# uber-research/UPSNet

Hardware: AMD Instinct MI355X
Metric: images/sec (whole node), UPSNet-50 1024x2048 (higher is better)
Workload: dtype f32

## Files before the change

upsnet_amd/csrc/conv_wino36.hip:

```cpp
#include <cstdlib>
#include <type_traits>
#include "conv_params.h"
#include "upsnet_hip.h"

#define W36_TM 32
#define W36_TN 64
#define W36_PTS 36
#define W36_VBUF (W36_PTS * 4 * W36_TM * 16)
#define W36_BSTEP (2 * W36_TN * 16)
#define W36_STEPS (2 * W36_PTS)
#define W36_XCH (16 * W36_PTS * 64 * 4)
#define W36_RING 3

typedef unsigned w36_uintx4 __attribute__((ext_vector_type(4)));

#define W36_BT(D0, D1, D2, D3, D4, D5)                                                                               \
    {                                                                                                                \
        const float a0_ = D0, a1_ = D1, a2_ = D2, a3_ = D3, a4_ = D4, a5_ = D5;                                       \
        const float e1_ = __builtin_fmaf(-2.25f, a2_, a4_), o1_ = __builtin_fmaf(-2.25f, a1_, a3_);                   \
        const float e3_ = __builtin_fmaf(-0.5625f, a2_, a4_), o3_ = __builtin_fmaf(-0.5625f, a1_, a3_);               \
        D0 = __builtin_fmaf(1.265625f, a0_, __builtin_fmaf(-2.8125f, a2_, a4_));                                     \
        D1 = __builtin_fmaf(0.75f, o1_, e1_);                                                                        \
        D2 = __builtin_fmaf(-0.75f, o1_, e1_);                                                                       \
        D3 = __builtin_fmaf(1.5f, o3_, e3_);                                                                         \
        D4 = __builtin_fmaf(-1.5f, o3_, e3_);                                                                        \
        D5 = __builtin_fmaf(1.265625f, a1_, __builtin_fmaf(-2.8125f, a3_, a5_));                                     \
    }
#define W36_AT(M0, M1, M2, M3, M4, M5, Y0, Y1, Y2, Y3)                                                               \
    {                                                                                                                \
        const float s1_ = (M1) + (M2), d1_ = (M1) - (M2), s2_ = (M3) + (M4), d2_ = (M3) - (M4);                      \
        Y0 = ((M0) + s1_) + s2_;                                                                                     \
        Y1 = __builtin_fmaf(1.5f, d2_, 0.75f * d1_);                                                                 \
        Y2 = __builtin_fmaf(2.25f, s2_, 0.5625f * s1_);                                                              \
        Y3 = __builtin_fmaf(3.375f, d2_, __builtin_fmaf(0.421875f, d1_, (M5)));                                      \
    }

template <bool SK>
__global__ void __launch_bounds__(512, 1) conv_wino36_f32_kernel(const ConvParams p)
{
    extern __shared__ __attribute__((aligned(16))) unsigned char smem_raw[];
    const int tid = threadIdx.x, lane = tid & 63;
    const int wave = __builtin_amdgcn_readfirstlane(tid >> 6);
    const int cb = wave >> 2, pg = wave & 3;
    const int lhalf = lane >> 5, l32 = lane & 31;
    int m_t, n_t, kz = 0;
    {
        const int nt = p.n_tiles;
        const int per = (p.m_tiles + 7) >> 3;
        int bid = (int)blockIdx.x;
        if constexpr (SK) { const int base_grid = 8 * per * nt; kz = bid / base_grid; bid -= kz * base_grid; }
        const int q = bid >> 3;
        n_t = q % nt;
        const int local = q / nt;
        m_t = (bid & 7) * per + local;
        if (local >= per || m_t >= p.m_tiles) return;
    }
    int si = 0;
#pragma unroll
    for (int q = 1; q < CV_MAXSEG; ++q) if (q < p.nseg && m_t >= p.seg[q].tile_start) si = q;
    const ConvSeg sg = p.seg[si];
    const long p0 = (long)(m_t - sg.tile_start) * W36_TM;
    const int nslabs_all = p.Cin >> 4;
    const int s_first = SK ? (kz * nslabs_all) / p.ksplit : 0;
    const int nslabs = SK ? ((kz + 1) * nslabs_all) / p.ksplit - s_first : nslabs_all;
    const long HoWo = (long)sg.Ho * sg.Wo;

    const int ltile = tid >> 4, lch = tid & 15;
    int hrow0, wcol0;
    int hlo, hhi;
    unsigned tbase, nrmask = 0, ncmask = 0;
    bool lane_fix;
    {
        const long pp = p0 + ltile;
        const bool tile_ok = pp < sg.M;
        const long ppc = tile_ok ? pp : sg.M - 1;
        const int n = (int)(ppc / HoWo);
        const int rem = (int)(ppc - (long)n * HoWo);
        const int ty = rem / sg.Wo, tx = rem - ty * sg.Wo;
        const int h0 = 4 * ty - 1;
        hlo = n * sg.H; hhi = tile_ok ? hlo + sg.H : hlo;
        hrow0 = hlo + h0;
        wcol0 = 4 * tx - 1;
#pragma unroll
        for (int r = 0; r < 6; ++r) nrmask |= (h0 + r >= 0 && h0 + r < sg.H) ? 0u : (1u << r);
#pragma unroll
        for (int c = 0; c < 6; ++c) ncmask |= (wcol0 + c >= 0 && wcol0 + c < sg.W) ? 0u : (1u << c);
        lane_fix = tile_ok && (nrmask | ncmask) != 0;
        tbase = (unsigned)(hrow0 * sg.W + wcol0) * (4u * (unsigned)p.Cin) + 4u * (unsigned)lch;
    }
    const bool fix = __builtin_amdgcn_ballot_w64(lane_fix) != 0ull;
    bool risky;
    {
        const long plast = min(p0 + (long)W36_TM, sg.M) - 1;
        const long nl = plast / HoWo;
        const long tyl = (plast - nl * HoWo) / sg.Wo;
        risky = (nl * sg.H + 4 * tyl + 4) * (long)sg.W + 4L * sg.Wo >= (long)sg.N * sg.H * sg.W;
    }
    const unsigned cin4 = 4u * (unsigned)p.Cin;
    const unsigned rowpitch = (unsigned)sg.W * cin4;
    const unsigned cin4_s = __builtin_amdgcn_readfirstlane(cin4);
    const unsigned rowpitch_s = __builtin_amdgcn_readfirstlane((unsigned)sg.W) * cin4_s;
    const unsigned cbase = (unsigned)wcol0 * cin4 + 4u * (unsigned)lch;
#define W36_ROWOFF(R) (((unsigned)min(max(hrow0 + (R), hlo), max(hhi - 1, hlo)) * rowpitch) | ((hrow0 + (R) >= hlo && hrow0 + (R) < hhi) ? 0u : 0x80000000u))
    const size_t xaddr = reinterpret_cast<size_t>(sg.x);
    const unsigned xlo = __builtin_amdgcn_readfirstlane((unsigned)xaddr), xhi = __builtin_amdgcn_readfirstlane((unsigned)(xaddr >> 32));
    const unsigned xbytes = __builtin_amdgcn_readfirstlane((unsigned)(sg.N * sg.H * sg.W) * 4u * (unsigned)p.Cin - (SK ? (unsigned)s_first * 64u : 0u));
    const char *xbase = reinterpret_cast<const char *>(((size_t)xhi << 32) | xlo) + (SK ? (size_t)s_first * 64 : 0);
#define W36_SWZ(Q) ((((Q) & 1) << 2) | (((Q) >> 1) << 1))
    const unsigned st_base = (unsigned)((((lch >> 2) * W36_TM + (ltile ^ W36_SWZ(lch >> 2))) * 16) + (lch & 3) * 4);
    constexpr unsigned XI_PITCH = 4 * W36_TM * 16;
    const unsigned fr_base0 = (unsigned)((lhalf * W36_TM + (l32 ^ W36_SWZ(lhalf))) * 16) + (unsigned)pg * 9u * XI_PITCH;
    const unsigned fr_base1 = (unsigned)(((2 + lhalf) * W36_TM + (l32 ^ W36_SWZ(2 + lhalf))) * 16) + (unsigned)pg * 9u * XI_PITCH;
    const size_t waddr = reinterpret_cast<size_t>(p.w) + ((size_t)n_t * (size_t)nslabs_all + (size_t)s_first) * (W36_STEPS * W36_BSTEP);
    const unsigned wlo = __builtin_amdgcn_readfirstlane((unsigned)waddr), whi = __builtin_amdgcn_readfirstlane((unsigned)(waddr >> 32));
    const __amdgpu_buffer_rsrc_t wrsrc = __builtin_amdgcn_make_buffer_rsrc(reinterpret_cast<void *>(((size_t)whi << 32) | wlo), 0,
                                                                            nslabs * (int)(W36_STEPS * W36_BSTEP), 0x00020000);
    const unsigned b_lane = (unsigned)(lhalf * (W36_TN * 16) + (32 * cb + l32) * 16);
    const int gmax = nslabs * W36_STEPS - 1;

    floatx16 acc[9];
#pragma unroll
    for (int i = 0; i < 9; ++i)
#pragma unroll
        for (int r = 0; r < 16; ++r) acc[i][r] = 0.f;

    float ld[36];
    float4 breg[W36_RING];

#define W36_LOADROW_FAST(R, RS) { unsigned so_ = (unsigned)((R) ? (R) - 1 : 0) * rowpitch_s; asm volatile("" : "+s"(so_));              \
        ld[6 * (R)] = __uint_as_float(__builtin_amdgcn_raw_buffer_load_b32(RS, (R) ? tbase + rowpitch_s : tbase, so_, 0));               \
        _Pragma("unroll") for (int c_ = 1; c_ < 6; ++c_) ld[6 * (R) + c_] = __uint_as_float(__builtin_amdgcn_raw_buffer_load_b32(       \
            RS, ((R) ? tbase + rowpitch_s : tbase) + cin4_s, so_ + (unsigned)(c_ - 1) * cin4_s, 0)); }
#define W36_LOADROW_SAFE(R, RS) { unsigned cb_ = cbase; asm volatile("" : "+v"(cb_)); const unsigned rb_ = W36_ROWOFF(R) + cb_; _Pragma("unroll") for (int c_ = 0; c_ < 6; ++c_) \
        ld[6 * (R) + c_] = __uint_as_float(__builtin_amdgcn_raw_buffer_load_b32(RS, (rb_ + (unsigned)c_ * cin4) | ((ncmask << (30 - c_)) & 0x40000000u), 0, 0)); }
#define W36_FIXROW(R) if (fix) { asm volatile("" ::: "memory"); const unsigned bad_ = ((nrmask >> (R)) & 1u) ? 0x3fu : ncmask;           \
        _Pragma("unroll") for (int c_ = 0; c_ < 6; ++c_) ld[6 * (R) + c_] = ((bad_ >> c_) & 1u) ? 0.f : ld[6 * (R) + c_]; }
#define W36_ROWPASS(R) W36_BT(ld[6 * (R) + 0], ld[6 * (R) + 1], ld[6 * (R) + 2], ld[6 * (R) + 3], ld[6 * (R) + 4], ld[6 * (R) + 5])
#define W36_COLSTASH(J, SB)                                                                                           \
    {                                                                                                                 \
        float c0_ = ld[0 + (J)], c1_ = ld[6 + (J)], c2_ = ld[12 + (J)], c3_ = ld[18 + (J)], c4_ = ld[24 + (J)], c5_ = ld[30 + (J)]; \
        W36_BT(c0_, c1_, c2_, c3_, c4_, c5_)                                                                          \
        *reinterpret_cast<float *>(smem_raw + (SB) + (0 * 6 + (J)) * XI_PITCH) = c0_;                                 \
        *reinterpret_cast<float *>(smem_raw + (SB) + (1 * 6 + (J)) * XI_PITCH) = c1_;                                 \
        *reinterpret_cast<float *>(smem_raw + (SB) + (2 * 6 + (J)) * XI_PITCH) = c2_;                                 \
        *reinterpret_cast<float *>(smem_raw + (SB) + (3 * 6 + (J)) * XI_PITCH) = c3_;                                 \
        *reinterpret_cast<float *>(smem_raw + (SB) + (4 * 6 + (J)) * XI_PITCH) = c4_;                                 \
        *reinterpret_cast<float *>(smem_raw + (SB) + (5 * 6 + (J)) * XI_PITCH) = c5_;                                 \
    }
#define W36_BLOAD(SLOT, G) { const w36_uintx4 v_ = __builtin_amdgcn_raw_buffer_load_b128(wrsrc, b_lane, (unsigned)min((G), gmax) * W36_BSTEP, 0); \
        breg[SLOT] = make_float4(__uint_as_float(v_.x), __uint_as_float(v_.y), __uint_as_float(v_.z), __uint_as_float(v_.w)); }

#pragma unroll
    for (int u = 0; u < W36_RING; ++u) W36_BLOAD(u, 18 * pg + u)
    {
        const __amdgpu_buffer_rsrc_t xr = __builtin_amdgcn_make_buffer_rsrc(const_cast<char *>(xbase), 0, xbytes, 0x00020000);
#pragma unroll
        for (int r = 0; r < 6; ++r) { W36_LOADROW_SAFE(r, xr) }
#pragma unroll
        for (int r = 0; r < 6; ++r) { W36_ROWPASS(r) }
#pragma unroll
        for (int j = 0; j < 6; ++j) { W36_COLSTASH(j, st_base) }
    }
    __syncthreads();
    float4 afr = *reinterpret_cast<const float4 *>(smem_raw + fr_base0);

    auto slab_loop = [&](auto fast_tag) __attribute__((always_inline)) {
    constexpr bool FAST = decltype(fast_tag)::value;
    for (int s = 0; s < nslabs; ++s) {
        const int sn = min(s + 1, nslabs - 1);
        const __amdgpu_buffer_rsrc_t xr = __builtin_amdgcn_make_buffer_rsrc(const_cast<char *>(xbase) + (size_t)sn * 64, 0, xbytes - (unsigned)sn * 64u, 0x00020000);
        const unsigned cur = (s & 1) ? W36_VBUF : 0u, nxt = W36_VBUF - cur;
        const unsigned sb = nxt + st_base;
        const int g0 = s * W36_STEPS + 18 * pg;
#pragma unroll
        for (int u = 0; u < 18; ++u) {
            if (u < 6) { if constexpr (FAST) { W36_LOADROW_FAST(u, xr) } else { W36_LOADROW_SAFE(u, xr) } }
            float4 afn;
            if (u < 17) afn = *reinterpret_cast<const float4 *>(smem_raw + cur + (((u + 1) & 1) ? fr_base1 : fr_base0) + (unsigned)((u + 1) >> 1) * XI_PITCH);
            else afn = *reinterpret_cast<const float4 *>(smem_raw + nxt + fr_base0);
            if (u == 6) { if constexpr (FAST) { W36_FIXROW(0) } W36_ROWPASS(0) }
            if (u == 7) { if constexpr (FAST) { W36_FIXROW(1) } W36_ROWPASS(1) }
            if (u == 8) { if constexpr (FAST) { W36_FIXROW(2) } W36_ROWPASS(2) }
            if (u == 9) { if constexpr (FAST) { W36_FIXROW(3) } W36_ROWPASS(3) }
            if (u == 10) { if constexpr (FAST) { W36_FIXROW(4) } W36_ROWPASS(4) }
            if (u == 11) { if constexpr (FAST) { W36_FIXROW(5) } W36_ROWPASS(5) W36_COLSTASH(0, sb) }
            if (u == 12) { W36_COLSTASH(1, sb) }
            if (u == 13) { W36_COLSTASH(2, sb) }
            if (u == 14) { W36_COLSTASH(3, sb) }
            if (u == 15) { W36_COLSTASH(4, sb) }
            if (u == 16) { W36_COLSTASH(5, sb) }
            const float4 bf = breg[u % W36_RING];
            acc[u >> 1] = __builtin_amdgcn_mfma_f32_32x32x2f32(afr.x, bf.x, acc[u >> 1], 0, 0, 0);
            acc[u >> 1] = __builtin_amdgcn_mfma_f32_32x32x2f32(afr.y, bf.y, acc[u >> 1], 0, 0, 0);
            acc[u >> 1] = __builtin_amdgcn_mfma_f32_32x32x2f32(afr.z, bf.z, acc[u >> 1], 0, 0, 0);
            acc[u >> 1] = __builtin_amdgcn_mfma_f32_32x32x2f32(afr.w, bf.w, acc[u >> 1], 0, 0, 0);
            W36_BLOAD(u % W36_RING, (u + W36_RING < 18 ? g0 : g0 + W36_STEPS - 18) + u + W36_RING)
            if (u == 16) __syncthreads();
            afr = afn;
            __builtin_amdgcn_sched_barrier(0);
        }
    }
    };
    if (risky) slab_loop(std::false_type{}); else slab_loop(std::true_type{});
#undef W36_LOADROW_FAST
#undef W36_LOADROW_SAFE
#undef W36_ROWOFF
#undef W36_FIXROW
#undef W36_ROWPASS
#undef W36_COLSTASH
#undef W36_BLOAD

    const unsigned crow = (unsigned)p.Cout * 4u;
    const size_t oaddr_ = reinterpret_cast<size_t>(SK ? p.partial + (size_t)kz * (size_t)p.m_total * (size_t)p.Cout : sg.out);
    const unsigned obytes_ = __builtin_amdgcn_readfirstlane((unsigned)((long)sg.N * sg.OH * sg.OW) * crow);
    const __amdgpu_buffer_rsrc_t orsrc = __builtin_amdgcn_make_buffer_rsrc(
        reinterpret_cast<void *>(((size_t)(unsigned)__builtin_amdgcn_readfirstlane((unsigned)(oaddr_ >> 32)) << 32) | (unsigned)__builtin_amdgcn_readfirstlane((unsigned)oaddr_)),
        0, (int)obytes_, 0x00020000);
    float *xch = reinterpret_cast<float *>(smem_raw);
#pragma unroll 1
    for (int bb = 0; bb < 2; ++bb) {
        __syncthreads();
        if (cb == bb) {
#pragma unroll
            for (int u = 0; u < 9; ++u)
#pragma unroll
                for (int r = 0; r < 16; ++r) xch[(r * W36_PTS + 9 * pg + u) * 64 + lane] = acc[u][r];
        }
        __syncthreads();
        const int co_ch = n_t * W36_TN + 32 * bb + l32;
        const bool co_ok = co_ch < p.Cout;
        const float bv = (p.bias != nullptr && co_ok) ? p.bias[co_ch] : 0.f;
#pragma unroll 1
        for (int rr = 0; rr < 2; ++rr) {
            const int r = 2 * wave + rr;
            const long pp = p0 + 8 * (r >> 2) + 4 * lhalf + (r & 3);
            float m[36];
#pragma unroll
            for (int x = 0; x < 36; ++x) m[x] = xch[(r * W36_PTS + x) * 64 + lane];
            if (!(co_ok && pp < sg.M)) continue;
            const int n = (int)(pp / HoWo);
            const int rem = (int)(pp - (long)n * HoWo);
            const int ty = rem / sg.Wo, tx = rem - ty * sg.Wo;
            float t[6][4];
#pragma unroll
            for (int i = 0; i < 6; ++i) W36_AT(m[6 * i + 0], m[6 * i + 1], m[6 * i + 2], m[6 * i + 3], m[6 * i + 4], m[6 * i + 5], t[i][0], t[i][1], t[i][2], t[i][3])
#pragma unroll
            for (int c = 0; c < 4; ++c) {
                float y[4];
                W36_AT(t[0][c], t[1][c], t[2][c], t[3][c], t[4][c], t[5][c], y[0], y[1], y[2], y[3])
                const int ox = 4 * tx + c;
#pragma unroll
                for (int a = 0; a < 4; ++a) {
                    const int oy = 4 * ty + a;
                    float v = y[a];
                    if constexpr (!SK) { v = v + bv; if (p.relu) v = fmaxf(v, 0.f); }
                    const unsigned off = (oy < sg.OH && ox < sg.OW) ? (unsigned)((n * sg.OH + oy) * sg.OW + ox) * crow + 4u * (unsigned)co_ch : 0x80000000u;
                    __builtin_amdgcn_raw_buffer_store_b32(__float_as_uint(v), orsrc, off, 0, 0);
                }
            }
        }
    }
}

static int w36_fill(ConvParams &p, const char *who, int nseg, const float *const x[], float *const out[], const int batch[], const int height[],
                    const int width[], int Cin, int Cout, const float *wpack, int ldw, const float *bias, int relu)
{
    UPS_REQUIRE(Cin > 0 && Cin % 32 == 0 && ldw % W36_TN == 0, "%s: Cin %% 32 == 0 and ldw %% 64 == 0 (got %d, %d)", who, Cin, ldw);
    int rc = conv_fill(p, who, nseg, x, nullptr, nullptr, nullptr, out, batch, height, width, Cin, Cout, wpack, ldw, bias, 3, 3, 1, 1, 1, relu);
    if (rc) return rc;
    UPS_REQUIRE((long)W36_PTS * Cin * ldw < (1L << 29), "%s: packed weight exceeds 2 GiB", who);
    int tiles = 0;
    for (int i = 0; i < nseg; ++i) {
        ConvSeg &s = p.seg[i];
        s.OH = s.Ho; s.OW = s.Wo;
        s.Ho = (s.OH + 3) / 4; s.Wo = (s.OW + 3) / 4;
        s.M = (long)s.N * s.Ho * s.Wo;
        UPS_REQUIRE((long)s.N * s.H * s.W * Cin < (1L << 28), "%s: feature map %d exceeds 1 GiB; split the batch", who, i);
        UPS_REQUIRE((long)s.N * s.OH * s.OW * Cout < (1L << 29), "%s: output %d exceeds 2 GiB; split the batch", who, i);
        s.tile_start = tiles;
        tiles += (int)((s.M + W36_TM - 1) / W36_TM);
    }
    p.m_tiles = tiles;
    p.n_tiles = ldw / W36_TN;
    return 0;
}

extern "C" int upsnet_conv2d_winograd36_nhwc_f32(void *stream, int nseg, const float *const x[], float *const out[], const int batch[],
                                                 const int height[], const int width[], int Cin, const float *wpack, int ldw, const float *bias,
                                                 int Cout, int relu)
{
    ConvParams p;
    int rc = w36_fill(p, "conv2d_winograd36_nhwc_f32", nseg, x, out, batch, height, width, Cin, Cout, wpack, ldw, bias, relu);
    if (rc) return rc;
    static std::atomic<unsigned long long> attr_dev{0};
    UPS_ONCE_PER_DEVICE(attr_dev, UPS_CHECK_HIP(hipFuncSetAttribute(reinterpret_cast<const void *>(&conv_wino36_f32_kernel<false>), hipFuncAttributeMaxDynamicSharedMemorySize, W36_XCH)));
    const int grid = 8 * ((p.m_tiles + 7) / 8) * p.n_tiles;
    hipLaunchKernelGGL(conv_wino36_f32_kernel<false>, dim3(grid), dim3(512), W36_XCH, (hipStream_t)stream, p);
    UPS_CHECK_LAUNCH("conv_wino36_f32_kernel");
    ups_set_form("wino36<%d,%d>", W36_TM, W36_TN);
    return 0;
}

extern "C" size_t upsnet_conv2d_winograd36_splitk_workspace_bytes(int batch, int height, int width, int Cout, int ksplit)
{
    return (size_t)ksplit * (size_t)batch * height * width * Cout * sizeof(float);
}

extern "C" int upsnet_conv2d_winograd36_nhwc_f32_splitk(void *stream, const float *x, float *out, int batch, int height, int width, int Cin,
                                                        const float *wpack, int ldw, const float *bias, int Cout, int relu, int ksplit,
                                                        void *workspace)
{
    const float *xs[1] = {x};
    float *os[1] = {out};
    const int nb[1] = {batch}, hh[1] = {height}, ww[1] = {width};
    ConvParams p;
    int rc = w36_fill(p, "conv2d_winograd36_nhwc_f32_splitk", 1, xs, os, nb, hh, ww, Cin, Cout, wpack, ldw, bias, relu);
    if (rc) return rc;
    UPS_REQUIRE(workspace && ksplit >= 2 && ksplit <= 8 && Cin / 16 >= ksplit, "conv2d_winograd36_nhwc_f32_splitk: ksplit 2..8, <= Cin / 16, and a workspace");
    p.ksplit = ksplit;
    p.partial = (float *)workspace;
    p.m_total = (long)batch * height * width;
    UPS_REQUIRE(p.m_total * Cout < (1L << 29), "conv2d_winograd36_nhwc_f32_splitk: output exceeds 2 GiB; split the batch");
    static std::atomic<unsigned long long> attr_dev{0};
    UPS_ONCE_PER_DEVICE(attr_dev, UPS_CHECK_HIP(hipFuncSetAttribute(reinterpret_cast<const void *>(&conv_wino36_f32_kernel<true>), hipFuncAttributeMaxDynamicSharedMemorySize, W36_XCH)));
    const int grid = 8 * ((p.m_tiles + 7) / 8) * p.n_tiles * ksplit;
    hipLaunchKernelGGL(conv_wino36_f32_kernel<true>, dim3(grid), dim3(512), W36_XCH, (hipStream_t)stream, p);
    UPS_CHECK_LAUNCH("conv_wino36_f32_kernel<splitk>");
    ups_set_form("wino36<%d,%d> splitk%d", W36_TM, W36_TN, ksplit);
    return conv_splitk_reduce((hipStream_t)stream, p.partial, ksplit, p.m_total, p.m_total, Cout, bias, nullptr, relu, out);
}

__global__ void conv_pack_weight_wino36_kernel(const float *__restrict__ w, int cout, int cin, int ldw, float *__restrict__ wp)
{
    const long total = (long)ldw * cin;
    const int nslabs = cin >> 4;
    const double G[6][3] = {{64.0 / 81, 0.0, 0.0}, {-128.0 / 243, -32.0 / 81, -8.0 / 27}, {-128.0 / 243, 32.0 / 81, -8.0 / 27},
                            {32.0 / 243, 16.0 / 81, 8.0 / 27}, {32.0 / 243, -16.0 / 81, 8.0 / 27}, {0.0, 0.0, 1.0}};
    for (long idx = (long)blockIdx.x * blockDim.x + threadIdx.x; idx < total; idx += (long)blockDim.x * gridDim.x) {
        const int co = idx % ldw, c = idx / ldw;
        double g[3][3], t[6][3];
#pragma unroll
        for (int a = 0; a < 3; ++a)
#pragma unroll
            for (int b = 0; b < 3; ++b) g[a][b] = co < cout ? (double)w[(((long)co * cin + c) * 3 + a) * 3 + b] : 0.0;
#pragma unroll
        for (int i = 0; i < 6; ++i)
#pragma unroll
            for (int b = 0; b < 3; ++b) t[i][b] = G[i][0] * g[0][b] + G[i][1] * g[1][b] + G[i][2] * g[2][b];
        const long blk = ((long)(co / W36_TN) * nslabs + (c >> 4)) * W36_PTS;
        const int q = (c & 15) >> 2, ci = c & 3, cl = co % W36_TN;
#pragma unroll
        for (int i = 0; i < 6; ++i)
#pragma unroll
            for (int j = 0; j < 6; ++j) {
                const double u = t[i][0] * G[j][0] + t[i][1] * G[j][1] + t[i][2] * G[j][2];
                wp[(((blk + i * 6 + j) * 4 + q) * W36_TN + cl) * 4 + ci] = (float)u;
            }
    }
}

extern "C" int upsnet_conv_pack_weight_winograd36(void *stream, const float *weight, int cout, int cin, int ldw, float *wpack)
{
    UPS_REQUIRE(weight && wpack && cout > 0 && cin > 0 && ldw >= cout, "conv_pack_weight_winograd36: bad args");
    UPS_REQUIRE(cin % 16 == 0 && ldw % W36_TN == 0, "conv_pack_weight_winograd36: Cin %% 16 must be 0 and ldw a multiple of 64");
    const long total = (long)ldw * cin;
    int blocks = (int)((total + 255) / 256);
    if (blocks > 65535) blocks = 65535;
    hipLaunchKernelGGL(conv_pack_weight_wino36_kernel, dim3(blocks), dim3(256), 0, (hipStream_t)stream, weight, cout, cin, ldw, wpack);
    UPS_CHECK_LAUNCH("conv_pack_weight_wino36_kernel");
    return 0;
}
```

Baseline: 172.4.

## Restructure Winograd epilogue exchange layout, vectorize LDS traffic, use fast prologue loads

Reworks the output-transform epilogue: accumulators are written to LDS as float4 in a new interleaved layout, then read as float2 pairs so each lane handles two adjacent tiles. Tile index math is done once and incremented, and store offsets are hoisted per row. The prologue now uses the fast input-load path when the tile is not risky, and the column stash splits its high rows into a separate base address. The aim is fewer LDS instructions, less integer division, and cheaper address math, in exchange for higher register pressure and more complex indexing.

```diff
diff --git a/upsnet_amd/csrc/conv_wino36.hip b/upsnet_amd/csrc/conv_wino36.hip
--- a/upsnet_amd/csrc/conv_wino36.hip
+++ b/upsnet_amd/csrc/conv_wino36.hip
@@ -13,6 +13,7 @@
 #define W36_RING 3
 
 typedef unsigned w36_uintx4 __attribute__((ext_vector_type(4)));
+typedef float w36_floatx2 __attribute__((ext_vector_type(2)));
 
 #define W36_BT(D0, D1, D2, D3, D4, D5)                                                                               \
     {                                                                                                                \
@@ -136,7 +137,7 @@
 #define W36_FIXROW(R) if (fix) { asm volatile("" ::: "memory"); const unsigned bad_ = ((nrmask >> (R)) & 1u) ? 0x3fu : ncmask;           \
         _Pragma("unroll") for (int c_ = 0; c_ < 6; ++c_) ld[6 * (R) + c_] = ((bad_ >> c_) & 1u) ? 0.f : ld[6 * (R) + c_]; }
 #define W36_ROWPASS(R) W36_BT(ld[6 * (R) + 0], ld[6 * (R) + 1], ld[6 * (R) + 2], ld[6 * (R) + 3], ld[6 * (R) + 4], ld[6 * (R) + 5])
-#define W36_COLSTASH(J, SB)                                                                                           \
+#define W36_COLSTASH(J, SB, SBH)                                                                                      \
     {                                                                                                                 \
         float c0_ = ld[0 + (J)], c1_ = ld[6 + (J)], c2_ = ld[12 + (J)], c3_ = ld[18 + (J)], c4_ = ld[24 + (J)], c5_ = ld[30 + (J)]; \
         W36_BT(c0_, c1_, c2_, c3_, c4_, c5_)                                                                          \
@@ -144,8 +145,8 @@
         *reinterpret_cast<float *>(smem_raw + (SB) + (1 * 6 + (J)) * XI_PITCH) = c1_;                                 \
         *reinterpret_cast<float *>(smem_raw + (SB) + (2 * 6 + (J)) * XI_PITCH) = c2_;                                 \
         *reinterpret_cast<float *>(smem_raw + (SB) + (3 * 6 + (J)) * XI_PITCH) = c3_;                                 \
-        *reinterpret_cast<float *>(smem_raw + (SB) + (4 * 6 + (J)) * XI_PITCH) = c4_;                                 \
-        *reinterpret_cast<float *>(smem_raw + (SB) + (5 * 6 + (J)) * XI_PITCH) = c5_;                                 \
+        *reinterpret_cast<float *>(smem_raw + (SBH) + (J) * XI_PITCH) = c4_;                                          \
+        *reinterpret_cast<float *>(smem_raw + (SBH) + (6 + (J)) * XI_PITCH) = c5_;                                    \
     }
 #define W36_BLOAD(SLOT, G) { const w36_uintx4 v_ = __builtin_amdgcn_raw_buffer_load_b128(wrsrc, b_lane, (unsigned)min((G), gmax) * W36_BSTEP, 0); \
         breg[SLOT] = make_float4(__uint_as_float(v_.x), __uint_as_float(v_.y), __uint_as_float(v_.z), __uint_as_float(v_.w)); }
@@ -154,12 +155,20 @@
     for (int u = 0; u < W36_RING; ++u) W36_BLOAD(u, 18 * pg + u)
     {
         const __amdgpu_buffer_rsrc_t xr = __builtin_amdgcn_make_buffer_rsrc(const_cast<char *>(xbase), 0, xbytes, 0x00020000);
-#pragma unroll
-        for (int r = 0; r < 6; ++r) { W36_LOADROW_SAFE(r, xr) }
+        if (risky) {
+#pragma unroll
+            for (int r = 0; r < 6; ++r) { W36_LOADROW_SAFE(r, xr) }
+        } else {
+#pragma unroll
+            for (int r = 0; r < 6; ++r) { W36_LOADROW_FAST(r, xr) }
+#pragma unroll
+            for (int r = 0; r < 6; ++r) { W36_FIXROW(r) }
+        }
 #pragma unroll
         for (int r = 0; r < 6; ++r) { W36_ROWPASS(r) }
-#pragma unroll
-        for (int j = 0; j < 6; ++j) { W36_COLSTASH(j, st_base) }
+        const unsigned st_hi = st_base + 24u * XI_PITCH;
+#pragma unroll
+        for (int j = 0; j < 6; ++j) { W36_COLSTASH(j, st_base, st_hi) }
     }
     __syncthreads();
     float4 afr = *reinterpret_cast<const float4 *>(smem_raw + fr_base0);
@@ -171,6 +180,8 @@
         const __amdgpu_buffer_rsrc_t xr = __builtin_amdgcn_make_buffer_rsrc(const_cast<char *>(xbase) + (size_t)sn * 64, 0, xbytes - (unsigned)sn * 64u, 0x00020000);
         const unsigned cur = (s & 1) ? W36_VBUF : 0u, nxt = W36_VBUF - cur;
         const unsigned sb = nxt + st_base;
+        unsigned sbh = sb + 24u * XI_PITCH;
+        asm volatile("" : "+v"(sbh));
         const int g0 = s * W36_STEPS + 18 * pg;
 #pragma unroll
         for (int u = 0; u < 18; ++u) {
@@ -183,12 +194,12 @@
             if (u == 8) { if constexpr (FAST) { W36_FIXROW(2) } W36_ROWPASS(2) }
             if (u == 9) { if constexpr (FAST) { W36_FIXROW(3) } W36_ROWPASS(3) }
             if (u == 10) { if constexpr (FAST) { W36_FIXROW(4) } W36_ROWPASS(4) }
-            if (u == 11) { if constexpr (FAST) { W36_FIXROW(5) } W36_ROWPASS(5) W36_COLSTASH(0, sb) }
-            if (u == 12) { W36_COLSTASH(1, sb) }
-            if (u == 13) { W36_COLSTASH(2, sb) }
-            if (u == 14) { W36_COLSTASH(3, sb) }
-            if (u == 15) { W36_COLSTASH(4, sb) }
-            if (u == 16) { W36_COLSTASH(5, sb) }
+            if (u == 11) { if constexpr (FAST) { W36_FIXROW(5) } W36_ROWPASS(5) W36_COLSTASH(0, sb, sbh) }
+            if (u == 12) { W36_COLSTASH(1, sb, sbh) }
+            if (u == 13) { W36_COLSTASH(2, sb, sbh) }
+            if (u == 14) { W36_COLSTASH(3, sb, sbh) }
+            if (u == 15) { W36_COLSTASH(4, sb, sbh) }
+            if (u == 16) { W36_COLSTASH(5, sb, sbh) }
             const float4 bf = breg[u % W36_RING];
             acc[u >> 1] = __builtin_amdgcn_mfma_f32_32x32x2f32(afr.x, bf.x, acc[u >> 1], 0, 0, 0);
             acc[u >> 1] = __builtin_amdgcn_mfma_f32_32x32x2f32(afr.y, bf.y, acc[u >> 1], 0, 0, 0);
@@ -216,46 +227,62 @@
     const __amdgpu_buffer_rsrc_t orsrc = __builtin_amdgcn_make_buffer_rsrc(
         reinterpret_cast<void *>(((size_t)(unsigned)__builtin_amdgcn_readfirstlane((unsigned)(oaddr_ >> 32)) << 32) | (unsigned)__builtin_amdgcn_readfirstlane((unsigned)oaddr_)),
         0, (int)obytes_, 0x00020000);
-    float *xch = reinterpret_cast<float *>(smem_raw);
-#pragma unroll 1
+    const unsigned crow_s = __builtin_amdgcn_readfirstlane(crow);
+    const unsigned opitch_s = __builtin_amdgcn_readfirstlane((unsigned)sg.OW) * crow_s;
+    constexpr unsigned XU = 64 * 16;
+    const int xh = (wave & 1) ^ ((lane >> 4) & 1);
+    const unsigned rd_base = (unsigned)(wave >> 1) * (W36_PTS * XU) + (unsigned)lane * 16u + 8u * (unsigned)xh;
+    const unsigned wr_base = 9u * (unsigned)pg * XU + (unsigned)lane * 16u;
+    const int M_i = (int)sg.M, HoWo_i = (int)HoWo;
+    int Wo_e = sg.Wo;
+    asm volatile("" : "+s"(Wo_e));
+#pragma unroll
     for (int bb = 0; bb < 2; ++bb) {
         __syncthreads();
         if (cb == bb) {
 #pragma unroll
-            for (int u = 0; u < 9; ++u)
-#pragma unroll
-                for (int r = 0; r < 16; ++r) xch[(r * W36_PTS + 9 * pg + u) * 64 + lane] = acc[u][r];
+            for (int rq = 0; rq < 4; ++rq)
+#pragma unroll
+                for (int u = 0; u < 9; ++u)
+                    *reinterpret_cast<float4 *>(smem_raw + wr_base + (unsigned)(rq * W36_PTS + u) * XU) = make_float4(acc[u][4 * rq], acc[u][4 * rq + 1], acc[u][4 * rq + 2], acc[u][4 * rq + 3]);
         }
         __syncthreads();
         const int co_ch = n_t * W36_TN + 32 * bb + l32;
         const bool co_ok = co_ch < p.Cout;
-        const float bv = (p.bias != nullptr && co_ok) ? p.bias[co_ch] : 0.f;
-#pragma unroll 1
+        float bv = 0.f;
+        if constexpr (!SK) bv = (p.bias != nullptr && co_ok) ? p.bias[co_ch] : 0.f;
+        float t[2][6][4];
+#pragma unroll
+        for (int i = 0; i < 6; ++i) {
+            w36_floatx2 v[6];
+#pragma unroll
+            for (int j = 0; j < 6; ++j) v[j] = *(const volatile __attribute__((address_space(3))) w36_floatx2 *)(smem_raw + rd_base + (unsigned)(6 * i + j) * XU);
+            W36_AT(v[0].x, v[1].x, v[2].x, v[3].x, v[4].x, v[5].x, t[0][i][0], t[0][i][1], t[0][i][2], t[0][i][3])
+            W36_AT(v[0].y, v[1].y, v[2].y, v[3].y, v[4].y, v[5].y, t[1][i][0], t[1][i][1], t[1][i][2], t[1][i][3])
+        }
+        int pp = (int)p0 + 8 * (wave >> 1) + 4 * lhalf + 2 * xh;
+        int n = pp / HoWo_i;
+        int ty, tx;
+        { const int rem = pp - n * HoWo_i; ty = rem / Wo_e; tx = rem - ty * Wo_e; }
+#pragma unroll
         for (int rr = 0; rr < 2; ++rr) {
-            const int r = 2 * wave + rr;
-            const long pp = p0 + 8 * (r >> 2) + 4 * lhalf + (r & 3);
-            float m[36];
-#pragma unroll
-            for (int x = 0; x < 36; ++x) m[x] = xch[(r * W36_PTS + x) * 64 + lane];
-            if (!(co_ok && pp < sg.M)) continue;
-            const int n = (int)(pp / HoWo);
-            const int rem = (int)(pp - (long)n * HoWo);
-            const int ty = rem / sg.Wo, tx = rem - ty * sg.Wo;
-            float t[6][4];
-#pragma unroll
-            for (int i = 0; i < 6; ++i) W36_AT(m[6 * i + 0], m[6 * i + 1], m[6 * i + 2], m[6 * i + 3], m[6 * i + 4], m[6 * i + 5], t[i][0], t[i][1], t[i][2], t[i][3])
+            if (rr) { ++pp; if (++tx == Wo_e) { tx = 0; if (++ty == sg.Ho) { ty = 0; ++n; } } }
+            const bool ok = co_ok && pp < M_i;
+            const unsigned obase = (unsigned)((n * sg.OH + 4 * ty) * sg.OW + 4 * tx) * crow + 4u * (unsigned)co_ch;
+            const int nrow = ok ? sg.OH - 4 * ty : 0, ncol = sg.OW - 4 * tx;
+            unsigned rowv[4];
+#pragma unroll
+            for (int a = 0; a < 4; ++a) rowv[a] = a < nrow ? obase + (unsigned)a * opitch_s : 0x80000000u;
 #pragma unroll
             for (int c = 0; c < 4; ++c) {
                 float y[4];
-                W36_AT(t[0][c], t[1][c], t[2][c], t[3][c], t[4][c], t[5][c], y[0], y[1], y[2], y[3])
-                const int ox = 4 * tx + c;
+                W36_AT(t[rr][0][c], t[rr][1][c], t[rr][2][c], t[rr][3][c], t[rr][4][c], t[rr][5][c], y[0], y[1], y[2], y[3])
+                const bool cok = c < ncol;
 #pragma unroll
                 for (int a = 0; a < 4; ++a) {
-                    const int oy = 4 * ty + a;
                     float v = y[a];
                     if constexpr (!SK) { v = v + bv; if (p.relu) v = fmaxf(v, 0.f); }
-                    const unsigned off = (oy < sg.OH && ox < sg.OW) ? (unsigned)((n * sg.OH + oy) * sg.OW + ox) * crow + 4u * (unsigned)co_ch : 0x80000000u;
-                    __builtin_amdgcn_raw_buffer_store_b32(__float_as_uint(v), orsrc, off, 0, 0);
+                    __builtin_amdgcn_raw_buffer_store_b32(__float_as_uint(v), orsrc, cok ? rowv[a] : 0x80000000u, (unsigned)c * crow_s, 0);
                 }
             }
         }
```

Result: no change. 172.6 (median of 6 runs) (+0.1%).
